# wkvong/multimodal-baby

Measured on AMD Instinct MI355X. Metric: image-text pairs/sec, CVCL ResNeXt+embed 224², bs256, 1/2/4/8 MI355X, higher is better.
Workload: dtype bf16; 1 GPU; C2 = BASELINE configs[1]: CVCL saycam_contrastive, frozen random-init ResNeXt-50 32x4d (BN train mode) + embedding mean-pool text encoder, E=512, L2-normalised, fixed tau 0.07, 224x224 frames + 3-word utterances; full step = fwd + InfoNCE + bwd(fc, embedding) + AdamW; per_gpu_batch=256, global_batch=256, negatives=local (single GPU), parallelism=dp1, trunk_streams=2

## Files before the change

include/cvcl_hip.h:

```cpp
#ifndef CVCL_HIP_H
#define CVCL_HIP_H

#include <stddef.h>
#include <stdint.h>

#ifdef __cplusplus
extern "C" {
#endif

#define CVCL_ABI_VERSION 7

enum { CVCL_OK = 0, CVCL_EINVAL = -1, CVCL_ELAUNCH = -2, CVCL_EWORKSPACE = -3, CVCL_EUNSUPPORTED = -4 };
enum { CVCL_F32 = 0, CVCL_BF16 = 1, CVCL_F32X3 = 2 };
enum { CVCL_ACT_NONE = 0, CVCL_ACT_RELU = 1, CVCL_ACT_GELU = 2, CVCL_ACT_QUICK_GELU = 3 };
#define CVCL_STATS_ACCUMULATE (-1)

int cvcl_abi_version(void);
const char* cvcl_last_error(void);

enum { CVCL_K_GEMM = 0, CVCL_K_GCONV = 1, CVCL_K_STEM = 2, CVCL_K_BN_FINALIZE = 3, CVCL_K_BN_ADD_RELU = 4,
       CVCL_K_MAXPOOL = 5, CVCL_K_AVGPOOL = 6, CVCL_K_HEAD = 7, CVCL_K_OTHER = 8, CVCL_K_ATTENTION = 9,
       CVCL_K_LAYERNORM = 10, CVCL_K_LSTM = 11, CVCL_K_GEMM_F32 = 12, CVCL_K_BN_APPLY = 13, CVCL_K_BN_BWD = 14,
       CVCL_K_WGRAD = 15, CVCL_K_GEMM8W = 16, CVCL_K_GEMM_PRO = 17, CVCL_K_NCLASSES = 18 };
int cvcl_prof_enable(int on);
// ... 21 lines not shown
                             void* stream);

size_t cvcl_infonce_workspace_bytes(int N);
int cvcl_infonce_fwd(const float* logits, int N, float* scalars5, float* row_lse, float* col_lse,
                     void* workspace, size_t workspace_bytes, void* stream);
int cvcl_infonce_bwd(const float* logits, const float* row_lse, const float* col_lse, const float* d_loss,
                     float* d_logits, int N, void* stream);

int cvcl_row_entropy(const float* x, float* out, int R, int N, void* stream);

typedef struct {
    const void* A; const void* W; void* C;
    int M, N, K, lda, ldw, ldc;
    const float* a_scale; const float* a_shift; int a_relu;
    int gather_ho, gather_wo, gather_hi, gather_wi, gather_stride;
    const float* exp_scale; const float* bias; int act;
    const void* R; int ldr;
    float* stats; int stats_rows;
    const float* c_scale; const float* c_shift; const float* r_scale; const float* r_shift;
    void* C_pre; const void* G; int ldg;
    const float* centre;
    const void* A2; const void* W2; int K2, lda2, ldw2; const float* centre2;
    const float* ln_stats; const float* ln_colsum; float* row_part;
    int a_trans, w_trans; float* a_rowsum;
    int f32_split;
} cvcl_gemm_args;
int cvcl_gemm_grid_m(int dtype, int M, int N, int has_prologue);
int cvcl_gemm(int dtype, const cvcl_gemm_args* args, void* stream);
int cvcl_gemm_stats_rows(int dtype, const cvcl_gemm_args* args);
int cvcl_gemm8w(int epi, const cvcl_gemm_args* args, void* stream);
int cvcl_gemm_pro(const cvcl_gemm_args* args, void* stream);
int cvcl_gemm_pro_supported(const cvcl_gemm_args* args);
int cvcl_gemm_pro_stats_rows(int M, int N);
int cvcl_gemm8w_supported(int M, int N, int K, int lda, int ldw, int ldc);
int cvcl_set_gemm_cu_share(int cus);
int cvcl_gemm_ln_supported(const cvcl_gemm_args* args);
int cvcl_row_stats(int dtype, const void* x, long x_row_stride, float* out, long rows, int D, float eps, void* stream);
int cvcl_row_stats_finalize(const float* row_part, int strips, float* out, long rows, int D, float eps, void* stream);
int cvcl_gemm8w_tile_rows(int M, int N);
int cvcl_gemm8w_stats_rows(int M, int N);

size_t cvcl_conv1x1_gram_workspace_bytes(int K);
int cvcl_conv1x1_gram(const void* A, int lda, long M, int K, const float* a_scale, const float* a_shift, int a_relu, void* workspace,
                      size_t workspace_bytes, const double** gram_out, void* stream);
int cvcl_bn_from_gram(const double* gram, int K, long count, const void* W, int ldw, int N, const float* gamma, const float* beta,
                      float* running_mean, float* running_var, int64_t* num_batches_tracked, float momentum, float eps,
                      float* scale, float* shift, float* moments, int moments_ld, const float* centre, void* stream);

int cvcl_transpose_f32(const float* in, float* out, int rows, int cols, void* stream);
int cvcl_colsum_f32(const float* dY, float* d_bias, int M, int N, void* stream);

enum { CVCL_PACK_DENSE = 0, CVCL_PACK_STEM7 = 1, CVCL_PACK_GCONV3 = 2 };

typedef struct {
    const void* w;
    const float* gamma; const float* beta;
    float* running_mean; float* running_var; int64_t* num_batches_tracked;
} cvcl_convbn_params;

int cvcl_bn_finalize(const float* stats, int rows, long count, const float* gamma, const float* beta,
                     float* running_mean, float* running_var, int64_t* num_batches_tracked, float momentum,
                     float eps, float* scale, float* shift, const float* centre, int C, void* stream);
int cvcl_bn_eval_affine(const float* gamma, const float* beta, const float* running_mean, const float* running_var,
                        float eps, float* scale, float* shift, const float* centre, int C, void* stream);
int cvcl_col_stats_rows(long rows);
int cvcl_col_stats(int dtype, const void* x, long rows, int C, float* stats, int stats_rows, void* stream);

size_t cvcl_packed_weight_bytes(int dtype, int kind, int cout, int cin_per_group, int k);
int cvcl_pack_conv_weight(int dtype, int kind, const float* w_oihw, void* out, int cout, int cin_per_group, int k,
                          void* stream);

int cvcl_stem_conv_stats_rows(int dtype, int B, int H, int W);
int cvcl_stem_conv7x7(int dtype, const float* x_nchw, const void* w_packed, void* y_nhwc, float* stats, int stats_rows,
                      const float* centre , int B, int H, int W, void* stream);
int cvcl_stem_pool_supported(int dtype, int H, int W);
int cvcl_stem_pool(int dtype, const float* x_nchw, const void* w_packed, const float* scale, const float* shift,
                   const float* centre , void* y_nhwc, int B, int H, int W, void* stream);
int cvcl_bn_relu_maxpool(int dtype, const void* x, const float* scale, const float* shift, void* y, int B, int H, int W,
                         int C, void* stream);
int cvcl_gconv3x3_stats_rows(int dtype, int B, int H, int W, int C, int stride);
int cvcl_gconv3x3(int dtype, const void* x, const float* a_scale, const float* a_shift, const void* w_packed, void* y,
                  float* stats, int stats_rows, const float* centre , int B, int H, int W, int C, int groups,
                  int stride, void* stream);
int cvcl_bn_add_relu(int dtype, const void* raw, const float* scale, const float* shift, const void* idn,
                     const float* idn_scale, const float* idn_shift, void* out, long rows, int C, void* stream);
int cvcl_bn_relu_apply(int dtype, const void* x, const float* scale, const float* shift, void* y, long rows, int C,
                       void* stream);
int cvcl_avgpool(int dtype, const void* x, float* out, int B, int HW, int C, void* stream);

size_t cvcl_resnext50_workspace_bytes(int dtype, int B, int H, int W);
size_t cvcl_resnext50_centres_floats(void);
int cvcl_resnext50_fwd(int dtype, int B, int H, int W, int training, const float* x_nchw,
                       const cvcl_convbn_params* layers, int n_layers, void* workspace, size_t workspace_bytes,
                       void* layer4_out_nhwc, float* pooled, float momentum, float eps, const float* centres, void* stream);
size_t cvcl_resnext50_block_workspace_bytes(int dtype, int B, int h, int w, int stage);
int cvcl_resnext50_block_fwd(int dtype, int B, int h, int w, int stage, int first, int training, const void* x_nhwc,
                             const cvcl_convbn_params* layers, int n_layers, void* workspace, size_t workspace_bytes,
                             void* out_nhwc, float momentum, float eps, const float* centres ,
                             void* stream);
size_t cvcl_resnext50_moments_floats(void);
int cvcl_resnext50_fwd_deferred_stats(int dtype, int B, int H, int W, const float* x_nchw,
                                      const cvcl_convbn_params* layers, int n_layers, void* workspace, size_t workspace_bytes,
                                      void* layer4_out_nhwc, float* pooled, float eps, float* moments, const float* centres,
                                      void* stream);
int cvcl_resnext50_apply_moments(const cvcl_convbn_params* layers, int n_layers, const float* moments, float momentum,
                                 void* stream);
size_t cvcl_resnext50_fwd_grouped_workspace_bytes(int dtype, int B, int H, int W, int group);
int cvcl_resnext50_fwd_grouped(int dtype, int B, int H, int W, int group, const float* x_nchw,
                               const cvcl_convbn_params* layers, int n_layers, void* workspace, size_t workspace_bytes,
                               void* layer4_out_nhwc, float* pooled, float eps, void* stream);

int cvcl_im2col_patches(int dtype, const float* x_nchw, void* cols, int B, int H, int W, int patch, int Kpad,
                        void* stream);
int cvcl_vit_assemble_tokens(int dtype, const void* tok, const float* cls, const float* pos, void* h, int B, int T,
                             int D, void* stream);
int cvcl_layernorm(int dtype, const void* x, long x_row_stride, const float* gamma, const float* beta, float eps,
                   void* y, int y_is_f32, long rows, int D, void* stream);
int cvcl_attention(int dtype, const void* qkv, const int64_t* key_tok, void* out, int B, int T, int heads, int head_dim,
                   float scale, void* stream);
int cvcl_attention_causal(int dtype, const void* qkv, void* out, int B, int T, int heads, int head_dim, float scale, void* stream);
int cvcl_clip_text_pool(const float* x, const int64_t* tok, const float* gamma, const float* beta, float eps, float* out, int B, int L,
                        int W, void* stream);
int cvcl_attention_mx(const void* qkv, void* out8, void* out_block_scales, int B, int T, int heads, int head_dim, float scale,
                      void* stream);
int cvcl_attention_train(const void* qkv, void* out, float* lse, int B, int T, int heads, int head_dim, float scale, void* stream);
int cvcl_attention_bwd(const void* qkv, const void* o, const void* d_o, const float* lse, void* d_qkv, int B, int T, int heads,
                       int head_dim, float scale, void* stream);
int cvcl_layernorm_bwd_rows_partials(long rows);
int cvcl_layernorm_bwd_rows(const void* x, long x_row_stride, const float* gamma, const void* dy, int dy_is_f32, long dy_row_stride,
                            float eps, const void* add, void* dx, long dx_row_stride, float* partial, long rows, int D, void* stream);
int cvcl_gelu_bf16(const void* u, const void* d_y, void* y, long n, void* stream);
int cvcl_vit_tokens_bwd(const void* dh, void* d_tok, float* d_pos, int B, int T, int D, void* stream);
int cvcl_attention_train_f32(const float* qkv, float* out, float* lse, int B, int T, int heads, int head_dim, float scale, void* stream);
int cvcl_attention_bwd_f32(const float* qkv, const float* o, const float* d_o, const float* lse, float* d_qkv, int B, int T, int heads,
                           int head_dim, float scale, void* stream);
int cvcl_layernorm_bwd_rows_f32(const float* x, long x_row_stride, const float* gamma, const float* dy, long dy_row_stride, float eps,
                                const float* add, float* dx, long dx_row_stride, float* partial, long rows, int D, void* stream);
int cvcl_gelu_f32(const float* u, const float* d_y, float* y, long n, void* stream);
int cvcl_vit_tokens_bwd_f32(const float* dh, float* d_tok, float* d_pos, int B, int T, int D, void* stream);
int cvcl_embed_gather_pos(const float* table, const int64_t* tok, const float* pos, float* x, int B, int L, int E, int V,
                          void* stream);
int cvcl_seq_sum_div(const float* x, const int64_t* len, float* ret, int B, int L, int E, void* stream);
int cvcl_lstm_cell(const float* gates, const int64_t* len, int t, float* h, float* c, float* out, int B, int L, int Hd,
                   void* stream);

int cvcl_dropout(const float* x, const float* residual, float* y, long n, float p, unsigned long long seed,
                 long shared_period, long inner, void* stream);
int cvcl_layernorm_bwd(const float* x, const float* gamma, const float* dy, float eps, float* dx, float* dy_xhat, long rows,
                       int D, void* stream);
int cvcl_relu_bwd(const float* y, const float* dy, float* dx, long n, void* stream);
int cvcl_embed_rows_bwd(const float* dx, const int64_t* tok, float* d_table, int n_pos, int E, int V, void* stream);
int cvcl_seq_sum_div_bwd(const float* d_ret, const int64_t* len, float* dx, int B, int L, int E, void* stream);
int cvcl_attention_small(const float* qkv, const int64_t* key_tok, const float* d_out, float* out, float* d_qkv, int B,
                         int T, int heads, int head_dim, float scale, float dropout_p, unsigned long long seed,
                         void* stream);
int cvcl_lstm_cell_train(const float* gates, const int64_t* len, int t, float* h, float* c, float* out ,
                         float* gates_act, float* c_save, float* h_prev_save, int B, int L, int Hd, void* stream);
int cvcl_lstm_cell_bwd(const float* gates_act, const float* c_save, const int64_t* len, int t, const float* dh, float* dc,
                       float* d_gates, float* dh_carry, int B, int L, int Hd, void* stream);

int cvcl_bn_apply(int dtype, const void* x, const float* scale, const float* shift, void* y, long rows, int C, int relu,
                  void* stream);
int cvcl_bn_bwd_partial_rows(int dtype, long rows, int C);
int cvcl_bn_bwd(int dtype, int mode, const void* x, const void* out, const void* dy, const float* scale, const float* shift,
                const float* mean, const float* rstd, const float* gamma, float* dgamma, float* dbeta, void* dx, void* g_out,
                long rows, int C, float* partial, int partial_rows, float* coef, void* stream);
// ... 138 lines not shown
```

multimodal-baby_amd/csrc/resnext.hip:

```cpp
#include <algorithm>
#include <array>
#include <cstdlib>
#include <type_traits>

#include "cvcl_common.h"

namespace {

constexpr int kMaxStatsRows = 1024;
constexpr size_t kTrunkAccLayer = (size_t)kBnAccRows * 2 * 2048;


__global__ __launch_bounds__(1024) void bn_finalize_kernel(const float* __restrict__ stats, int rows, double count,
                                                           const float* __restrict__ gamma, const float* __restrict__ beta,
                                                           float* __restrict__ running_mean, float* __restrict__ running_var,
                                                           int64_t* __restrict__ nbt, float momentum, float eps,
                                                           float* __restrict__ scale, float* __restrict__ shift, int C,
                                                           float* __restrict__ moments, int moments_ld,
                                                           const float* __restrict__ centre) {
    constexpr int NS = 64, NC = 16;
    __shared__ double ps[NS][NC], pq[NS][NC];
    const int c = threadIdx.x & (NC - 1), sl = threadIdx.x / NC, ch = blockIdx.x * NC + c;
    double s = 0.0, q = 0.0;
    if (ch < C) {
// ... 663 lines not shown
    f32x4 acc_init = {0.f, 0.f, 0.f, 0.f};
    if (p.centre) {
        const f32x4 cv = *reinterpret_cast<const f32x4*>(p.centre + c0 + wave * 16 + kb * 4);
        acc_init = f32x4{-cv[0], -cv[1], -cv[2], -cv[3]};
    }
    const int n_items = p.B * p.bands;
    const int st_off = (tid >> 3) * p.C + (tid & 7) * 8;
    __builtin_amdgcn_s_waitcnt(0x0F70);
    const int bx = (gridDim.x & 7) == 0 ? (int)((blockIdx.x & 7) * (gridDim.x >> 3) + (blockIdx.x >> 3)) : (int)blockIdx.x;
    if (bx < n_items) prefetch(bx);
    for (int item = bx; item < n_items; item += gridDim.x) {
        const int b = item / p.bands, band = item - b * p.bands;
        const int oy0 = band * p.TH;
        __syncthreads();
        auto stage = [&](auto RELU) __attribute__((always_inline)) {
#pragma unroll
            for (int i = 0; i < NPF; ++i) {
                const int pi = s_pix0 + 32 * i;
                const unsigned keep = pf_in[i] ? 0xffffffffu : 0u;
                u32x4 v;
#pragma unroll
                for (int e = 0; e < 4; ++e) {
                    unsigned y = round2(__builtin_elementwise_fma(widen2(pf[i][e]), sc[e], sh[e]));
                    if constexpr (decltype(RELU)::value) y = relu2(y);
                    v[e] = y & keep;
                }
                if (pi < npix_in) *reinterpret_cast<u32x4*>(smem + pi * GC_PIXB + s_chunk * 16) = v;
            }
        };
        if (relu_in) stage(std::true_type{});
        else stage(std::false_type{});
        __syncthreads();
        if (item + (int)gridDim.x < n_items) prefetch(item + gridDim.x);
        const int rows_left = p.Ho - oy0;
#pragma unroll
        for (int mt = 0; mt < NMT; mt += 2) {
            if (mt >= n_mt) break;
            const int e0 = mtab[mt], e1 = mtab[mt + 1];
            const int base0 = e0 & 0xffff, base1 = e1 & 0xffff;
            const int q0 = pix + 16 * mt, q1 = q0 + 16;
            const bool wr0 = (e0 >> 24) && ((e0 >> 16) & 0xff) < rows_left, wr1 = (e1 >> 24) && ((e1 >> 16) & 0xff) < rows_left;
            f32x4 acc0 = acc_init, acc1 = acc_init;
#pragma unroll
            for (int ks = 0; ks < KS; ++ks) {
                const bf16x8 a0 = *reinterpret_cast<const bf16x8*>(smem + base0 + tap_off[ks]);
                const bf16x8 a1 = *reinterpret_cast<const bf16x8*>(smem + base1 + tap_off[ks]);
                acc0 = __builtin_amdgcn_mfma_f32_16x16x32_bf16(wf[ks], a0, acc0, 0, 0, 0);
                acc1 = __builtin_amdgcn_mfma_f32_16x16x32_bf16(wf[ks], a1, acc1, 0, 0, 0);
            }
            if (wr0) {
                const u32x2 o = {round2(f32x2{acc0[0], acc0[1]}), round2(f32x2{acc0[2], acc0[3]})};
                *reinterpret_cast<u32x2*>(s_out + q0 * GC_PIXB + wave * 32 + kb * 8) = o;
#pragma unroll
                for (int e = 0; e < 2; ++e) { const f32x2 sv = widen2(o[e]); ssum[e] += sv; ssq[e] = __builtin_elementwise_fma(sv, sv, ssq[e]); }
            }
            if (wr1) {
                const u32x2 o = {round2(f32x2{acc1[0], acc1[1]}), round2(f32x2{acc1[2], acc1[3]})};
                *reinterpret_cast<u32x2*>(s_out + q1 * GC_PIXB + wave * 32 + kb * 8) = o;
#pragma unroll
                for (int e = 0; e < 2; ++e) { const f32x2 sv = widen2(o[e]); ssum[e] += sv; ssq[e] = __builtin_elementwise_fma(sv, sv, ssq[e]); }
            }
        }
        __syncthreads();
        const int valid_rows = min(p.TH, p.Ho - oy0);
        const int n_chunks = valid_rows * p.Wo * 8;
        bf16_t* yb = y + ((long)b * p.Ho + oy0) * p.Wo * p.C + c0 + st_off;
        const char* so = s_out + (tid >> 3) * GC_PIXB + (tid & 7) * 16;
#pragma unroll
        for (int k = 0; k < NMT / 2; ++k) {
            if (tid + 256 * k < n_chunks)
                *reinterpret_cast<bf16x8*>(yb + (long)k * 32 * p.C) = *reinterpret_cast<const bf16x8*>(so + k * 32 * GC_PIXB);
        }
    }
#pragma unroll
    for (int e = 0; e < 4; ++e) {
        float s = ssum[e >> 1][e & 1], q = ssq[e >> 1][e & 1];
#pragma unroll
        for (int o = 1; o < 16; o <<= 1) { s += __shfl_xor(s, o, 64); q += __shfl_xor(q, o, 64); }
        if (pix == 0 && p.stats) {
            const int ch = c0 + wave * 16 + kb * 4 + e;
            cvcl_bn_stats_out(p.stats, p.stats_acc, blockIdx.x, p.C, ch, s, q);
        }
    }
}

__global__ __launch_bounds__(256) void gconv_direct_f32_kernel(const float* __restrict__ x, const float* __restrict__ a_scale,
                                                               const float* __restrict__ a_shift, const float* __restrict__ w,
                                                               float* __restrict__ y, const float* __restrict__ centre,
                                                               int B, int H, int W, int C, int cg,
                                                               int stride, int Ho, int Wo, float act_floor) {
    const long total = (long)B * Ho * Wo * C;
    for (long i = (long)blockIdx.x * blockDim.x + threadIdx.x; i < total; i += (long)gridDim.x * blockDim.x) {
        const int co = (int)(i % C);
        const long pp = i / C;
        const int ox = (int)(pp % Wo), oy = (int)((pp / Wo) % Ho), b = (int)(pp / ((long)Wo * Ho));
        const int g0 = (co / cg) * cg;
        float acc = centre ? -centre[co] : 0.f;
        for (int ci = 0; ci < cg; ++ci) {
            const float sc = a_scale ? a_scale[g0 + ci] : 1.f, sh = a_scale ? a_shift[g0 + ci] : 0.f;
            for (int ky = 0; ky < 3; ++ky) {
                const int yin = oy * stride - 1 + ky;
                if (yin < 0 || yin >= H) continue;
                for (int kx = 0; kx < 3; ++kx) {
                    const int xin = ox * stride - 1 + kx;
                    if (xin < 0 || xin >= W) continue;
                    const float v = fmaxf(fmaf(x[(((long)b * H + yin) * W + xin) * C + g0 + ci], sc, sh), act_floor);
                    acc = fmaf(v, w[((long)co * cg + ci) * 9 + ky * 3 + kx], acc);
                }
            }
        }
        y[i] = acc;
    }
}

template <int CG>
__global__ __launch_bounds__(256) void gconv_tiled_f32_kernel(const float* __restrict__ x, const float* __restrict__ a_scale,
                                                              const float* __restrict__ a_shift, const float* __restrict__ w,
                                                              float* __restrict__ y, const float* __restrict__ centre,
                                                              int B, int H, int W, int C, int stride, int Ho, int Wo, int TH,
                                                              int bands, int plane_p, float act_floor) {
    extern __shared__ __attribute__((aligned(16))) float smf[];
    constexpr int NG = 64 / CG;
    const int Wp = W + 2, rows_in = (TH - 1) * stride + 3, plane = rows_in * Wp;
    float* ws = smf;
    float* cs = ws + 64 * 9 * CG;
    float* xs = cs + 64;
    const int c0 = blockIdx.y * 64;
    const int tid = threadIdx.x, lane = tid & 63;
    const int wave = __builtin_amdgcn_readfirstlane(tid >> 6);
    for (int e = tid; e < 64 * CG * 9; e += 256) {
        const int co = e / (CG * 9), r = e - co * (CG * 9), ci = r / 9, tap = r - ci * 9;
        const int g = co / CG, o = co - g * CG;
        ws[((g * 9 + tap) * CG + ci) * CG + o] = w[(long)c0 * CG * 9 + e];
    }
    if (tid < 64) cs[tid] = centre ? -centre[c0 + tid] : 0.f;
    const int ch4 = tid & 15;
    f32x4 sc4 = {1.f, 1.f, 1.f, 1.f}, sh4 = {0.f, 0.f, 0.f, 0.f};
    if (a_scale) {
        sc4 = *reinterpret_cast<const f32x4*>(a_scale + c0 + ch4 * 4);
        sh4 = *reinterpret_cast<const f32x4*>(a_shift + c0 + ch4 * 4);
    }
    for (int item = blockIdx.x; item < B * bands; item += gridDim.x) {
        const int b = item / bands, band = item - b * bands;
        const int oy0 = band * TH, iy0 = oy0 * stride - 1;
        __syncthreads();
        for (int pix = tid >> 4; pix < plane; pix += 16) {
            const int ry = pix / Wp, rx = pix - ry * Wp;
            const int yin = iy0 + ry, xin = rx - 1;
            f32x4 v = {0.f, 0.f, 0.f, 0.f};
            if ((unsigned)yin < (unsigned)H && (unsigned)xin < (unsigned)W) {
                v = *reinterpret_cast<const f32x4*>(x + (((long)b * H + yin) * W + xin) * C + c0 + ch4 * 4);
                if (a_scale) {
#pragma unroll
                    for (int k = 0; k < 4; ++k) v[k] = fmaxf(fmaf(v[k], sc4[k], sh4[k]), act_floor);
                }
            }
#pragma unroll
            for (int k = 0; k < 4; ++k) xs[(ch4 * 4 + k) * plane_p + pix] = v[k];
        }
        __syncthreads();
        const int n_out = min(TH, Ho - oy0) * Wo, nblk = (n_out + 63) / 64;
        for (int u = wave; u < NG * nblk; u += 4) {
            const int g = u / nblk, blk = u - g * nblk;
            const int q = blk * 64 + lane;
            const bool ok = q < n_out;
            const int qq = ok ? q : 0, ty = qq / Wo, ox = qq - ty * Wo;
// ... 388 lines not shown
                       "cvcl_stem_conv7x7: width %d not supported by the staged patch", W);
        const int g = stem_grid(B, H);
        CVCL_CHECK_ARG(!stats || stats_rows >= g, "cvcl_stem_conv7x7: stats_rows %d < %d", stats_rows, g);
        const size_t lds = (size_t)3 * STEM_ROWS * STEM_PITCH * 4 + 4 * 16 * STEM_OPITCH + 64 * 4;
        float* st = stats;
        CVCL_CHECK_ARG(st, "cvcl_stem_conv7x7: the bf16 kernel always emits statistics; pass a buffer");
        CvclProfScope prof(stream, CVCL_K_STEM);
        hipLaunchKernelGGL(stem_mfma_kernel, dim3(g), dim3(256), lds, s, x_nchw, (const bf16_t*)w_packed, (bf16_t*)y_nhwc,
                           st, centre, B, H, W);
        CVCL_LAUNCH_CHECK();
        return CVCL_OK;
    }
    const long total = (long)B * (H / 2) * (W / 2) * 64;
    {
        CvclProfScope prof(stream, CVCL_K_STEM);
        const int Ho = H / 2;
        auto lds_of = [&](int th) { return (size_t)(147 * 64 + 64 + 3 * (2 * th + 5) * (W + 6)) * 4; };
        int TH = Ho < 8 ? Ho : 8;
        while (TH > 1 && lds_of(TH) > 150 * 1024) --TH;
        if (lds_of(TH) <= 150 * 1024) {
            static CvclLdsAttr attr;
            if (const int rc = cvcl_raise_lds_limit(attr, (const void*)stem_tiled_f32_kernel, 160 * 1024, "cvcl_stem_conv7x7")) return rc;
            attr.mark();
            const int bands = cvcl_div_up(Ho, TH);
            const long items = (long)B * bands;
            hipLaunchKernelGGL(stem_tiled_f32_kernel, dim3((unsigned)(items < 1024 ? items : 1024)), dim3(256), lds_of(TH), s, x_nchw,
                               (const float*)w_packed, (float*)y_nhwc, centre, B, H, W, TH, bands);
        } else {
            hipLaunchKernelGGL(stem_direct_f32_kernel, dim3(cvcl_grid(total, 256, 8192)), dim3(256), 0, s, x_nchw,
                               (const float*)w_packed, (float*)y_nhwc, centre, B, H, W);
        }
    }
    CVCL_LAUNCH_CHECK();
    if (stats) return cvcl_col_stats(CVCL_F32, y_nhwc, (long)B * (H / 2) * (W / 2), 64, stats, stats_rows, stream);
    return CVCL_OK;
}

extern "C" int cvcl_stem_pool_supported(int dtype, int H, int W) {
    return dtype == CVCL_BF16 && H % 2 == 0 && W % 4 == 0 && W / 4 <= 64 && W + 6 + 8 <= 2 * STEM_PITCH && W / 2 + 2 <= STEMP_BW;
}

extern "C" int cvcl_stem_pool(int dtype, const float* x_nchw, const void* w_packed, const float* scale, const float* shift,
                              const float* centre, void* y_nhwc, int B, int H, int W, void* stream) {
    CVCL_CHECK_DTYPE(dtype, "cvcl_stem_pool");
    CVCL_CHECK_ARG(x_nchw && w_packed && scale && shift && y_nhwc && B > 0, "cvcl_stem_pool: bad args");
    CVCL_CHECK_ARG(cvcl_stem_pool_supported(dtype, H, W), "cvcl_stem_pool: bf16 and a width <= %d only (got dtype %d, %d x %d)",
                   2 * (STEMP_BW - 2), dtype, H, W);
    const size_t lds = (size_t)3 * STEMP_ROWS * STEM_PITCH * 4 + (size_t)STEMP_CR * STEMP_BW * 128 + 3 * 64 * 4;
    static CvclLdsAttr attr;
    if (const int rc = cvcl_raise_lds_limit(attr, (const void*)stem_pool_mfma_kernel, (int)lds, "cvcl_stem_pool")) return rc;
    attr.mark();
    const int Hp = (H / 2 - 1) / 2 + 1;
    const int items = B * cvcl_div_up(Hp, STEMP_TP);
    int dev = 0, cus = 256;
    if (hipGetDevice(&dev) != hipSuccess || hipDeviceGetAttribute(&cus, hipDeviceAttributeMultiprocessorCount, dev) != hipSuccess || cus <= 0) cus = 256;
    const int grid = items < cus ? items : cus;
    CvclProfScope prof(stream, CVCL_K_STEM);
    hipLaunchKernelGGL(stem_pool_mfma_kernel, dim3(grid), dim3(512), lds, (hipStream_t)stream, x_nchw, (const bf16_t*)w_packed,
                       (bf16_t*)y_nhwc, scale, shift, centre, B, H, W);
    CVCL_LAUNCH_CHECK();
    return CVCL_OK;
}

extern "C" int cvcl_bn_relu_maxpool(int dtype, const void* x, const float* scale, const float* shift, void* y, int B,
                                    int H, int W, int C, void* stream) {
    CVCL_CHECK_DTYPE_TRUNK(dtype, "cvcl_bn_relu_maxpool");
    dtype = cvcl_storage_dtype(dtype);
    CVCL_CHECK_ARG(x && scale && shift && y && C % 8 == 0, "cvcl_bn_relu_maxpool: bad args");
    CvclProfScope prof(stream, CVCL_K_MAXPOOL);
    const int Ho = (H - 1) / 2 + 1, Wo = (W - 1) / 2 + 1;
    const long total = (long)B * ((Ho + POOL_ROWS - 1) / POOL_ROWS) * Wo * (C / 8);
    const int grid = cvcl_grid(total, 256, 8192);
    if (dtype == CVCL_F32)
        hipLaunchKernelGGL(bn_relu_maxpool_kernel<float>, dim3(grid), dim3(256), 0, (hipStream_t)stream,
                           (const float*)x, scale, shift, (float*)y, B, H, W, C);
    else
        hipLaunchKernelGGL(bn_relu_maxpool_kernel<bf16_t>, dim3(grid), dim3(256), 0, (hipStream_t)stream,
                           (const bf16_t*)x, scale, shift, (bf16_t*)y, B, H, W, C);
    CVCL_LAUNCH_CHECK();
    return CVCL_OK;
}

namespace {
struct GconvPlan { int TH, bands, rows_in, grid_x; size_t lds; };
GconvPlan gconv_plan(int B, int H, int W, int C, int stride) {
    GconvPlan g;
    const int Ho = (H - 1) / stride + 1, Wo = (W - 1) / stride + 1, Wp = W + 2;
    auto bytes = [&](int th) { return (size_t)(((th - 1) * stride + 3) * Wp + th * Wo) * GC_PIXB; };
    int TH = Ho;
    while (TH > 1 && (bytes(TH) > (size_t)52 * 1024 || ((TH - 1) * stride + 3) * Wp > 10 * 32 || TH * Wo > 128)) TH = (TH + 1) / 2;
    g.TH = TH;
    g.bands = cvcl_div_up(Ho, TH);
    g.rows_in = (TH - 1) * stride + 3;
    g.lds = bytes(TH);
    int per_cu = (int)((160 * 1024) / g.lds);
    const int reg_limit = (C / 32 == 32) ? 2 : 3;
    if (per_cu > reg_limit) per_cu = reg_limit;
    if (per_cu < 1) per_cu = 1;
    const int slabs = C / GC_CS;
    int gx = per_cu * 256 / slabs;
    if (gx < 1) gx = 1;
    const int items = B * g.bands;
    g.grid_x = items < gx ? items : gx;
    return g;
}
}

extern "C" int cvcl_gconv3x3_stats_rows(int dtype, int B, int H, int W, int C, int stride) {
    if (!cvcl_dtype_trunk(dtype)) return 0;
    if (dtype == CVCL_F32X3) return C % 32 == 0 ? cvcl_gconv_split_stats_rows(B, H, W, C, stride) : 0;
    if (dtype == CVCL_BF16) return gconv_plan(B, H, W, C, stride).grid_x;
    const int Ho = (H - 1) / stride + 1, Wo = (W - 1) / stride + 1;
    return cvcl_col_stats_rows((long)B * Ho * Wo);
}

static int gconv3x3_impl(int dtype, const void* x, const float* a_scale, const float* a_shift, const BnSrc* src, const void* w_packed,
                         void* y, float* stats, int stats_rows, const float* centre, int B, int H, int W, int C, int groups,
                         int stride, void* stream) {
    CVCL_CHECK_DTYPE_TRUNK(dtype, "cvcl_gconv3x3");
    CVCL_CHECK_ARG(x && w_packed && y && (!a_scale == !a_shift), "cvcl_gconv3x3: null pointer");
    CVCL_CHECK_ARG(!src || (dtype == CVCL_BF16 && src->acc && src->gamma && src->beta && src->C == C && src->count > 0 &&
                            (const void*)src->acc != (const void*)stats),
                   "cvcl_gconv3x3: finalize-on-load source");
    CVCL_CHECK_ARG(stats_rows != CVCL_STATS_ACCUMULATE || dtype == CVCL_BF16, "cvcl_gconv3x3: accumulators exist for bf16 only");
    const float act_floor = (a_scale || src) ? 0.f : -INFINITY;
    CVCL_CHECK_ARG(B > 0 && (stride == 1 || stride == 2) && groups > 0 && C % groups == 0, "cvcl_gconv3x3: bad shape");
    const int cg = C / groups;
    const int Ho = (H - 1) / stride + 1, Wo = (W - 1) / stride + 1;
    hipStream_t s = (hipStream_t)stream;
    if (dtype == CVCL_F32X3)
        return cvcl_gconv_split((const float*)x, a_scale, a_shift, act_floor, w_packed, (float*)y, stats, stats_rows, centre, B, H, W, C,
                                cg, stride, stream);
    if (dtype == CVCL_BF16) {
        CVCL_CHECK_ARG((cg == 4 || cg == 8 || cg == 16 || cg == 32) && C % GC_CS == 0,
                       "cvcl_gconv3x3: unsupported channels-per-group %d (C=%d)", cg, C);
        const GconvPlan g = gconv_plan(B, H, W, C, stride);
        CVCL_CHECK_ARG(g.lds <= 160 * 1024 && g.rows_in * (W + 2) <= 10 * 32 && g.TH * ((W - 1) / stride + 1) <= 128,
                       "cvcl_gconv3x3: feature map too wide for one staged band (%zu B, %d pixels)", g.lds, g.rows_in * (W + 2));
        CVCL_CHECK_ARG(!stats || stats_rows == CVCL_STATS_ACCUMULATE || stats_rows >= g.grid_x, "cvcl_gconv3x3: stats_rows %d < %d", stats_rows, g.grid_x);
        GconvDev d;
        d.x = x; d.a_scale = a_scale; d.a_shift = a_shift; d.w = w_packed; d.y = y; d.stats = stats; d.centre = centre;
        d.B = B; d.H = H; d.W = W; d.C = C; d.cg = cg; d.stride = stride; d.Ho = Ho; d.Wo = Wo;
        d.TH = g.TH; d.bands = g.bands; d.rows_in = g.rows_in;
        d.act_floor = act_floor;
        d.src = BnSrc{};
        d.stats_acc = stats && stats_rows == CVCL_STATS_ACCUMULATE;
        if (src) {
            CVCL_CHECK_ARG(g.lds >= 2048, "cvcl_gconv3x3: band buffers smaller than the finalize-on-load scratch");
            d.src = *src;
        }
        CvclProfScope prof(stream, CVCL_K_GCONV);
        int rc;
        const int slots = cvcl_div_up(g.rows_in * (W + 2), 32);
        static CvclLdsAttr attr_set[2][2][11];
        auto launch = [&](auto kern) -> int {
            CvclLdsAttr& done = attr_set[cg == 32][g.TH * Wo <= 64][slots <= 4 ? 4 : slots <= 6 ? 6 : slots <= 8 ? 8 : 10];
            if (const int rc = cvcl_raise_lds_limit(done, (const void*)kern, 160 * 1024, "cvcl_gconv3x3")) return rc;
            done.mark();
            hipLaunchKernelGGL(kern, dim3(g.grid_x, C / GC_CS), dim3(256), g.lds, s, d);
            return CVCL_OK;
        };
        const bool few = g.TH * Wo <= 64;
#define CVCL_GCONV_PICK(W_) \
        (slots <= 4 ? (few ? launch(gconv_mfma_kernel<W_, 4, 4>) : launch(gconv_mfma_kernel<W_, 4, 8>)) \
         : slots <= 6 ? (few ? launch(gconv_mfma_kernel<W_, 6, 4>) : launch(gconv_mfma_kernel<W_, 6, 8>)) \
         : slots <= 8 ? (few ? launch(gconv_mfma_kernel<W_, 8, 4>) : launch(gconv_mfma_kernel<W_, 8, 8>)) \
                      : (few ? launch(gconv_mfma_kernel<W_, 10, 4>) : launch(gconv_mfma_kernel<W_, 10, 8>)))
        rc = cg == 32 ? CVCL_GCONV_PICK(true) : CVCL_GCONV_PICK(false);
#undef CVCL_GCONV_PICK
        if (rc) return rc;
        CVCL_LAUNCH_CHECK();
        return CVCL_OK;
    }
    const long total = (long)B * Ho * Wo * C;
    {
        CvclProfScope prof(stream, CVCL_K_GCONV);
        auto plane_p_of = [&](int th) { const int pl = ((th - 1) * stride + 3) * (W + 2); return pl + ((9 - (pl & 7)) & 7); };
        auto lds_of = [&](int th) { return (size_t)(64 * 9 * cg + 64 + 64 * plane_p_of(th)) * 4; };
        int TH = Ho;
        while (TH > 1 && lds_of(TH) > 150 * 1024) --TH;
        const bool tiled = C % 64 == 0 && (cg == 4 || cg == 8 || cg == 16 || cg == 32) && lds_of(TH) <= 150 * 1024 &&
                           ((uintptr_t)x & 15) == 0 && ((uintptr_t)y & 15) == 0 && ((uintptr_t)a_scale & 15) == 0 && ((uintptr_t)a_shift & 15) == 0;
        if (tiled) {
            const int bands = cvcl_div_up(Ho, TH);
            const long items = (long)B * bands;
            const int slabs = C / 64;
            long gx = 1024 / slabs;
            if (gx < 1) gx = 1;
            if (gx > items) gx = items;
            static CvclLdsAttr attr[4];
            auto launch = [&](auto kern, int slot) -> int {
                if (const int rc = cvcl_raise_lds_limit(attr[slot], (const void*)kern, 160 * 1024, "cvcl_gconv3x3")) return rc;
                attr[slot].mark();
                hipLaunchKernelGGL(kern, dim3((unsigned)gx, slabs), dim3(256), lds_of(TH), s, (const float*)x, a_scale, a_shift,
                                   (const float*)w_packed, (float*)y, centre, B, H, W, C, stride, Ho, Wo, TH, bands, plane_p_of(TH), act_floor);
                return CVCL_OK;
            };
            const int rc = cg == 4 ? launch(gconv_tiled_f32_kernel<4>, 0) : cg == 8 ? launch(gconv_tiled_f32_kernel<8>, 1)
                         : cg == 16 ? launch(gconv_tiled_f32_kernel<16>, 2) : launch(gconv_tiled_f32_kernel<32>, 3);
            if (rc) return rc;
        } else {
            hipLaunchKernelGGL(gconv_direct_f32_kernel, dim3(cvcl_grid(total, 256, 8192)), dim3(256), 0, s, (const float*)x, a_scale,
                               a_shift, (const float*)w_packed, (float*)y, centre, B, H, W, C, cg, stride, Ho, Wo, act_floor);
        }
    }
    CVCL_LAUNCH_CHECK();
    if (stats) return cvcl_col_stats(CVCL_F32, y, (long)B * Ho * Wo, C, stats, stats_rows, stream);
    return CVCL_OK;
}

extern "C" int cvcl_gconv3x3(int dtype, const void* x, const float* a_scale, const float* a_shift, const void* w_packed,
                             void* y, float* stats, int stats_rows, const float* centre, int B, int H, int W, int C, int groups,
                             int stride, void* stream) {
    return gconv3x3_impl(dtype, x, a_scale, a_shift, nullptr, w_packed, y, stats, stats_rows, centre, B, H, W, C, groups, stride, stream);
}

extern "C" int cvcl_bn_add_relu(int dtype, const void* raw, const float* scale, const float* shift, const void* idn,
                                const float* idn_scale, const float* idn_shift, void* out, long rows, int C, void* stream) {
    CVCL_CHECK_DTYPE_TRUNK(dtype, "cvcl_bn_add_relu");
    dtype = cvcl_storage_dtype(dtype);
    CVCL_CHECK_ARG(raw && scale && shift && idn && out && rows > 0 && C % 8 == 0, "cvcl_bn_add_relu: bad args");
    CvclProfScope prof(stream, CVCL_K_BN_ADD_RELU);
    CVCL_CHECK_ARG((idn_scale == nullptr) == (idn_shift == nullptr), "cvcl_bn_add_relu: idn_scale/idn_shift pair");
    const int epc = dtype == CVCL_F32 ? 4 : 8;
    CVCL_CHECK_ARG(C % epc == 0, "cvcl_bn_add_relu: C must be a multiple of %d", epc);
    hipStream_t s = (hipStream_t)stream;
    const int cc = C / epc;
    int g256 = cc, t256 = 256;
    while (t256) { const int r = g256 % t256; g256 = t256; t256 = r; }
    const int mult = cc / g256;
    int grid = cvcl_grid(rows * (long)cc, 256 * 4, 16384);
    grid = (grid + mult - 1) / mult * mult;
    if (dtype == CVCL_F32)
        hipLaunchKernelGGL(bn_add_relu_kernel<float>, dim3(grid), dim3(256), 0, s, (const float*)raw,
                           scale, shift, (const float*)idn, idn_scale, idn_shift, (float*)out, rows, C);
    else
        hipLaunchKernelGGL(bn_add_relu_kernel<bf16_t>, dim3(grid), dim3(256), 0, s, (const bf16_t*)raw,
                           scale, shift, (const bf16_t*)idn, idn_scale, idn_shift, (bf16_t*)out, rows, C);
    CVCL_LAUNCH_CHECK();
    return CVCL_OK;
}

extern "C" int cvcl_bn_relu_apply(int dtype, const void* x, const float* scale, const float* shift, void* y, long rows,
                                  int C, void* stream) {
    CVCL_CHECK_DTYPE_TRUNK(dtype, "cvcl_bn_relu_apply");
    dtype = cvcl_storage_dtype(dtype);
    CVCL_CHECK_ARG(x && scale && shift && y && rows > 0, "cvcl_bn_relu_apply: bad args");
    CvclProfScope prof(stream, CVCL_K_BN_APPLY);
    const int epc = dtype == CVCL_F32 ? 4 : 8;
    CVCL_CHECK_ARG(C % epc == 0, "cvcl_bn_relu_apply: C must be a multiple of %d", epc);
    const int cc = C / epc;
    int g256 = cc, t256 = 256;
    while (t256) { const int r = g256 % t256; g256 = t256; t256 = r; }
    const int mult = cc / g256;
    int grid = cvcl_grid(rows * (long)cc, 256 * 4, 16384);
    grid = (grid + mult - 1) / mult * mult;
    if (dtype == CVCL_F32)
        hipLaunchKernelGGL(bn_relu_apply_kernel<float>, dim3(grid), dim3(256), 0, (hipStream_t)stream, (const float*)x, scale,
                           shift, (float*)y, rows, C);
    else
        hipLaunchKernelGGL(bn_relu_apply_kernel<bf16_t>, dim3(grid), dim3(256), 0, (hipStream_t)stream, (const bf16_t*)x,
                           scale, shift, (bf16_t*)y, rows, C);
    CVCL_LAUNCH_CHECK();
    return CVCL_OK;
}

extern "C" int cvcl_avgpool(int dtype, const void* x, float* out, int B, int HW, int C, void* stream) {
    CVCL_CHECK_DTYPE_TRUNK(dtype, "cvcl_avgpool");
    dtype = cvcl_storage_dtype(dtype);
    CVCL_CHECK_ARG(x && out && B > 0 && HW > 0 && C > 0, "cvcl_avgpool: bad args");
    CvclProfScope prof(stream, CVCL_K_AVGPOOL);
    if (dtype == CVCL_F32)
        hipLaunchKernelGGL(avgpool_kernel<float>, dim3(cvcl_grid((long)B * C, 256, 4096)), dim3(256), 0, (hipStream_t)stream, (const float*)x, out, B, HW, C);
    else
        hipLaunchKernelGGL(avgpool_kernel<bf16_t>, dim3(cvcl_grid((long)B * C, 256, 4096)), dim3(256), 0, (hipStream_t)stream, (const bf16_t*)x, out, B, HW, C);
    CVCL_LAUNCH_CHECK();
    return CVCL_OK;
}

namespace {
constexpr int kLayers[4] = {3, 4, 6, 3};
constexpr int kTrunkLayers = 53;
constexpr int kMaxC = 2048;
constexpr int kAffStride = 2 * kMaxC;
enum { kConv1, kConv2, kConv3, kDownsample };
static_assert(sizeof(EvalAffineAll::C) == sizeof(int) * kTrunkLayers && sizeof(ApplyMomentsAll::C) == sizeof(int) * kTrunkLayers,
              "the one-launch layer tables hold the whole trunk");

constexpr int block_layer_c(int stage, int j) { return (64 << stage) * (j < kConv3 ? 2 : 4); }

constexpr std::array<int, kTrunkLayers> kTrunkC = [] {
    std::array<int, kTrunkLayers> c = {64};
    int l = 1;
    for (int st = 0; st < 4; ++st)
        for (int b = 0; b < kLayers[st]; ++b)
            for (int j = 0; j < (b == 0 ? 4 : 3); ++j) c[l++] = block_layer_c(st, j);
    return c;
}();

// ... 454 lines not shown
```

Measured before the change: 51110 pairs/s.

## Add warp-specialized producer/consumer pipelined grouped 3x3 conv kernel

Adds a 512-thread grouped-conv kernel in which 256 threads load, apply the input BN affine, and stage the next band into double-buffered LDS, while the other 256 threads run MFMA on the current band and write outputs to a separate buffer that the producers store. It is chosen by default for stride-1 shapes 28/256, 14/512 and 7/1024. The intent is to overlap global loads and stores with MFMA compute and hide memory latency. In exchange the kernel needs more LDS per block, uses smaller bands, and allows fewer resident blocks per CU.

```diff
diff --git a/include/cvcl_hip.h b/include/cvcl_hip.h
--- a/include/cvcl_hip.h
+++ b/include/cvcl_hip.h
@@ -127,6 +127,12 @@
 int cvcl_gconv3x3(int dtype, const void* x, const float* a_scale, const float* a_shift, const void* w_packed, void* y,
                   float* stats, int stats_rows, const float* centre , int B, int H, int W, int C, int groups,
                   int stride, void* stream);
+int cvcl_gconv3x3_planned_form(int H, int W, int C, int stride);
+int cvcl_gconv3x3_form_stats_rows(int form, int B, int H, int W, int C, int stride);
+int cvcl_gconv3x3_form(int form, const void* x, const float* a_scale, const float* a_shift, const int64_t* src_acc,
+                       const float* src_gamma, const float* src_beta, double src_count, float src_eps, const void* w_packed, void* y,
+                       float* stats, int stats_rows, const float* centre , int B, int H, int W, int C, int groups,
+                       int stride, void* stream);
 int cvcl_bn_add_relu(int dtype, const void* raw, const float* scale, const float* shift, const void* idn,
                      const float* idn_scale, const float* idn_shift, void* out, long rows, int C, void* stream);
 int cvcl_bn_relu_apply(int dtype, const void* x, const float* scale, const float* shift, void* y, long rows, int C,
diff --git a/multimodal-baby_amd/csrc/resnext.hip b/multimodal-baby_amd/csrc/resnext.hip
--- a/multimodal-baby_amd/csrc/resnext.hip
+++ b/multimodal-baby_amd/csrc/resnext.hip
@@ -769,6 +769,210 @@
             cvcl_bn_stats_out(p.stats, p.stats_acc, blockIdx.x, p.C, ch, s, q);
         }
     }
+}
+
+__host__ __device__ constexpr int gcp_barriers(int n_items_of_workgroup) { return n_items_of_workgroup + 1; }
+constexpr int GCP_OUTB = 128;
+
+template <bool WIDE, int NMT>
+__device__ __forceinline__ void gcp_consumer(const GconvDev& p, char* smem, int tid, int bx, int n_local, int in_bytes, int out_bytes) {
+    const int lane = tid & 63, wave = tid >> 6;
+    const int pix = lane & 15, kb = lane >> 4;
+    const int c0 = blockIdx.y * GC_CS;
+    const int Wp = p.W + 2;
+    constexpr bool wide = WIDE;
+    constexpr int KS = WIDE ? 9 : 5;
+    const int unit = c0 / 16 + wave;
+    const bf16_t* wu = (const bf16_t*)p.w + (long)unit * KS * 512;
+    bf16x8 wf[KS];
+#pragma unroll
+    for (int ks = 0; ks < KS; ++ks) wf[ks] = *reinterpret_cast<const bf16x8*>(wu + (ks * 16 + pix) * 32 + kb * 8);
+    const int in_ch_off = wide ? ((wave >> 1) * 32 + kb * 8) : (wave * 16 + (kb & 1) * 8);
+    f32x2 ssum[2] = {f32x2{0.f, 0.f}, f32x2{0.f, 0.f}}, ssq[2] = {f32x2{0.f, 0.f}, f32x2{0.f, 0.f}};
+    const int n_out = p.TH * p.Wo, n_mt = cvcl_div_up(n_out, 16);
+    int tap_off[KS];
+#pragma unroll
+    for (int ks = 0; ks < KS; ++ks) {
+        int tap = wide ? ks : 2 * ks + (kb >> 1);
+        if (tap > 8) tap = 8;
+        const int ky = tap / 3, kx = tap - ky * 3;
+        tap_off[ks] = (ky * Wp + kx) * GC_PIXB + in_ch_off * 2;
+    }
+    int mtab[NMT];
+#pragma unroll
+    for (int mt = 0; mt < NMT; ++mt) {
+        const int q = pix + 16 * mt;
+        const bool ok = mt < n_mt && q < n_out;
+        const int ty = q / p.Wo, ox = q - ty * p.Wo;
+        mtab[mt] = ok ? ((((ty * p.stride) * Wp + ox * p.stride) * GC_PIXB) | (ty << 16) | (1 << 24)) : 0;
+    }
+    f32x4 acc_init = {0.f, 0.f, 0.f, 0.f};
+    if (p.centre) {
+        const f32x4 cv = *reinterpret_cast<const f32x4*>(p.centre + c0 + wave * 16 + kb * 4);
+        acc_init = f32x4{-cv[0], -cv[1], -cv[2], -cv[3]};
+    }
+    const int out_off = pix * GCP_OUTB + (((wave * 2 + (kb >> 1)) ^ ((pix >> 1) & 7)) << 4) + (kb & 1) * 8;
+    const int nb = gcp_barriers(n_local);
+    for (int j = 0; j < nb; ++j) {
+        if (j >= 1) {
+            const int k = j - 1, item = bx + k * (int)gridDim.x;
+            const int band = item % p.bands, oy0 = band * p.TH;
+            const char* s_in = smem + (k & 1) * in_bytes;
+            char* s_out = smem + 2 * in_bytes + (k & 1) * out_bytes + out_off;
+            const int rows_left = p.Ho - oy0;
+#pragma unroll
+            for (int mt = 0; mt < NMT; mt += 2) {
+                if (mt >= n_mt) break;
+                const int e0 = mtab[mt], e1 = mtab[mt + 1];
+                const int base0 = e0 & 0xffff, base1 = e1 & 0xffff;
+                const bool wr0 = (e0 >> 24) && ((e0 >> 16) & 0xff) < rows_left, wr1 = (e1 >> 24) && ((e1 >> 16) & 0xff) < rows_left;
+                f32x4 acc0 = acc_init, acc1 = acc_init;
+#pragma unroll
+                for (int ks = 0; ks < KS; ++ks) {
+                    const bf16x8 a0 = *reinterpret_cast<const bf16x8*>(s_in + base0 + tap_off[ks]);
+                    const bf16x8 a1 = *reinterpret_cast<const bf16x8*>(s_in + base1 + tap_off[ks]);
+                    acc0 = __builtin_amdgcn_mfma_f32_16x16x32_bf16(wf[ks], a0, acc0, 0, 0, 0);
+                    acc1 = __builtin_amdgcn_mfma_f32_16x16x32_bf16(wf[ks], a1, acc1, 0, 0, 0);
+                }
+                if (wr0) {
+                    const u32x2 o = {round2(f32x2{acc0[0], acc0[1]}), round2(f32x2{acc0[2], acc0[3]})};
+                    *reinterpret_cast<u32x2*>(s_out + 16 * mt * GCP_OUTB) = o;
+#pragma unroll
+                    for (int e = 0; e < 2; ++e) { const f32x2 sv = widen2(o[e]); ssum[e] += sv; ssq[e] = __builtin_elementwise_fma(sv, sv, ssq[e]); }
+                }
+                if (wr1) {
+                    const u32x2 o = {round2(f32x2{acc1[0], acc1[1]}), round2(f32x2{acc1[2], acc1[3]})};
+                    *reinterpret_cast<u32x2*>(s_out + 16 * (mt + 1) * GCP_OUTB) = o;
+#pragma unroll
+                    for (int e = 0; e < 2; ++e) { const f32x2 sv = widen2(o[e]); ssum[e] += sv; ssq[e] = __builtin_elementwise_fma(sv, sv, ssq[e]); }
+                }
+            }
+        }
+        __syncthreads();
+    }
+#pragma unroll
+    for (int e = 0; e < 4; ++e) {
+        float s = ssum[e >> 1][e & 1], q = ssq[e >> 1][e & 1];
+#pragma unroll
+        for (int o = 1; o < 16; o <<= 1) { s += __shfl_xor(s, o, 64); q += __shfl_xor(q, o, 64); }
+        if (pix == 0 && p.stats) {
+            const int ch = c0 + wave * 16 + kb * 4 + e;
+            cvcl_bn_stats_out(p.stats, p.stats_acc, blockIdx.x, p.C, ch, s, q);
+        }
+    }
+}
+
+template <int NPF, int NMT>
+__device__ __forceinline__ void gcp_producer(const GconvDev& p, char* smem, int tid, int bx, int n_local, int in_bytes, int out_bytes,
+                                             const float* aff) {
+    const bf16_t* __restrict__ x = (const bf16_t*)p.x;
+    bf16_t* __restrict__ y = (bf16_t*)p.y;
+    const int c0 = blockIdx.y * GC_CS;
+    const int Wp = p.W + 2;
+    const int s_chunk = tid & 7, s_pix0 = tid >> 3;
+    f32x2 sc[4], sh[4];
+#pragma unroll
+    for (int e = 0; e < 4; ++e) {
+        const int cl = s_chunk * 8 + 2 * e, ch = c0 + cl;
+        if (aff) {
+            sc[e] = f32x2{aff[cl], aff[cl + 1]};
+            sh[e] = f32x2{aff[64 + cl], aff[64 + cl + 1]};
+        } else {
+            sc[e] = p.a_scale ? f32x2{p.a_scale[ch], p.a_scale[ch + 1]} : f32x2{1.f, 1.f};
+            sh[e] = p.a_scale ? f32x2{p.a_shift[ch], p.a_shift[ch + 1]} : f32x2{0.f, 0.f};
+        }
+    }
+    const bool relu_in = p.act_floor == 0.f;
+    const int npix_in = p.rows_in * Wp;
+    u32x4 pf[NPF];
+    bool pf_in[NPF];
+    int slot_y[NPF], slot_xoff[NPF];
+    bool slot_ok[NPF];
+#pragma unroll
+    for (int i = 0; i < NPF; ++i) {
+        const int pi = s_pix0 + 32 * i;
+        const int pc = min(pi, npix_in - 1);
+        const int ry = pc / Wp, xin = pc - ry * Wp - 1;
+        slot_y[i] = ry;
+        slot_ok[i] = pi < npix_in && xin >= 0 && xin < p.W;
+        slot_xoff[i] = min(max(xin, 0), p.W - 1) * p.C;
+    }
+    const int row_elems = p.W * p.C;
+    auto prefetch = [&](int item) {
+        const int b = item / p.bands, band = item - b * p.bands;
+        const int iy0 = band * p.TH * p.stride - 1;
+        const bf16_t* xb = x + (long)b * p.H * p.W * p.C + c0 + s_chunk * 8;
+#pragma unroll
+        for (int i = 0; i < NPF; ++i) {
+            const int yin = iy0 + slot_y[i];
+            pf_in[i] = slot_ok[i] && (unsigned)yin < (unsigned)p.H;
+            const int yc = min(max(yin, 0), p.H - 1);
+            pf[i] = *reinterpret_cast<const u32x4*>(xb + (yc * row_elems + slot_xoff[i]));
+        }
+    };
+    auto stage = [&](char* s_in, auto RELU) __attribute__((always_inline)) {
+#pragma unroll
+        for (int i = 0; i < NPF; ++i) {
+            const int pi = s_pix0 + 32 * i;
+            const unsigned keep = pf_in[i] ? 0xffffffffu : 0u;
+            u32x4 v;
+#pragma unroll
+            for (int e = 0; e < 4; ++e) {
+                unsigned y = round2(__builtin_elementwise_fma(widen2(pf[i][e]), sc[e], sh[e]));
+                if constexpr (decltype(RELU)::value) y = relu2(y);
+                v[e] = y & keep;
+            }
+            if (pi < npix_in) *reinterpret_cast<u32x4*>(s_in + pi * GC_PIXB + s_chunk * 16) = v;
+        }
+    };
+    const int st_off = (tid >> 3) * p.C + (tid & 7) * 8;
+    const int so_off = (tid >> 3) * GCP_OUTB + (((tid & 7) ^ ((tid >> 4) & 7)) << 4);
+    auto store = [&](int k) {
+        const int item = bx + k * (int)gridDim.x;
+        const int b = item / p.bands, band = item - b * p.bands;
+        const int oy0 = band * p.TH;
+        const int valid_rows = min(p.TH, p.Ho - oy0);
+        const int n_chunks = valid_rows * p.Wo * 8;
+        bf16_t* yb = y + ((long)b * p.Ho + oy0) * p.Wo * p.C + c0 + st_off;
+        const char* so = smem + 2 * in_bytes + (k & 1) * out_bytes + so_off;
+#pragma unroll
+        for (int kk = 0; kk < NMT / 2; ++kk) {
+            if (tid + 256 * kk < n_chunks)
+                *reinterpret_cast<bf16x8*>(yb + (long)kk * 32 * p.C) = *reinterpret_cast<const bf16x8*>(so + kk * 32 * GCP_OUTB);
+        }
+    };
+    if (n_local > 0) prefetch(bx);
+    const int nb = gcp_barriers(n_local);
+    for (int j = 0; j < nb; ++j) {
+        if (j < n_local) {
+            char* s_in = smem + (j & 1) * in_bytes;
+            if (relu_in) stage(s_in, std::true_type{});
+            else stage(s_in, std::false_type{});
+            if (j + 1 < n_local) prefetch(bx + (j + 1) * (int)gridDim.x);
+        }
+        if (j >= 2) store(j - 2);
+        __syncthreads();
+    }
+    if (nb >= 2) store(nb - 2);
+}
+
+template <bool WIDE, int NPF, int NMT>
+__global__ __launch_bounds__(512, NPF <= 6 ? 4 : 2) void gconv_mfma_pipe_kernel(GconvDev p) {
+    extern __shared__ __attribute__((aligned(16))) char smem[];
+    const int tid = threadIdx.x;
+    const int c0 = blockIdx.y * GC_CS;
+    const float* aff = nullptr;
+    if (p.src.acc) {
+        float* a = reinterpret_cast<float*>(smem + 2 * p.rows_in * (p.W + 2) * GC_PIXB);
+        bn_slice_affine<GC_CS>(p.src, c0, blockIdx.x == 0, a, a + 64);
+        aff = a;
+    }
+    const int bx = (gridDim.x & 7) == 0 ? (int)((blockIdx.x & 7) * (gridDim.x >> 3) + (blockIdx.x >> 3)) : (int)blockIdx.x;
+    const int n_items = p.B * p.bands;
+    const int n_local = bx < n_items ? (n_items - bx + (int)gridDim.x - 1) / (int)gridDim.x : 0;
+    const int in_bytes = p.rows_in * (p.W + 2) * GC_PIXB, out_bytes = p.TH * p.Wo * GCP_OUTB;
+    if (tid < 256) gcp_consumer<WIDE, NMT>(p, smem, tid, bx, n_local, in_bytes, out_bytes);
+    else gcp_producer<NPF, NMT>(p, smem, tid - 256, bx, n_local, in_bytes, out_bytes, aff);
 }
 
 __global__ __launch_bounds__(256) void gconv_direct_f32_kernel(const float* __restrict__ x, const float* __restrict__ a_scale,
@@ -1323,19 +1527,28 @@
 }
 
 namespace {
-struct GconvPlan { int TH, bands, rows_in, grid_x; size_t lds; };
-GconvPlan gconv_plan(int B, int H, int W, int C, int stride) {
+enum { GCONV_ONE_PHASE = 0, GCONV_PIPELINED = 1, GCONV_FORM_OF_PLAN = -1 };
+struct GconvPlan { int TH, bands, rows_in, grid_x, form; size_t lds; };
+bool gconv_pipelined_wins(int H, int W, int C, int stride) {
+    return stride == 1 && H == W && ((H == 28 && C == 256) || (H == 14 && C == 512) || (H == 7 && C == 1024));
+}
+GconvPlan gconv_plan(int B, int H, int W, int C, int stride, int form = GCONV_FORM_OF_PLAN) {
     GconvPlan g;
     const int Ho = (H - 1) / stride + 1, Wo = (W - 1) / stride + 1, Wp = W + 2;
     auto bytes = [&](int th) { return (size_t)(((th - 1) * stride + 3) * Wp + th * Wo) * GC_PIXB; };
     int TH = Ho;
     while (TH > 1 && (bytes(TH) > (size_t)52 * 1024 || ((TH - 1) * stride + 3) * Wp > 10 * 32 || TH * Wo > 128)) TH = (TH + 1) / 2;
+    g.form = form == GCONV_FORM_OF_PLAN ? (gconv_pipelined_wins(H, W, C, stride) ? GCONV_PIPELINED : GCONV_ONE_PHASE) : form;
+    auto bytes_pipe = [&](int th) { return 2 * ((size_t)((th - 1) * stride + 3) * Wp * GC_PIXB + (size_t)th * Wo * GCP_OUTB); };
+    if (g.form == GCONV_PIPELINED)
+        while (TH > 1 && (bytes_pipe(TH) > (size_t)80 * 1024 || ((TH - 1) * stride + 3) * Wp > 6 * 32)) TH = (TH + 1) / 2;
     g.TH = TH;
     g.bands = cvcl_div_up(Ho, TH);
     g.rows_in = (TH - 1) * stride + 3;
-    g.lds = bytes(TH);
+    g.lds = g.form == GCONV_PIPELINED ? bytes_pipe(TH) : bytes(TH);
     int per_cu = (int)((160 * 1024) / g.lds);
-    const int reg_limit = (C / 32 == 32) ? 2 : 3;
+    const int reg_limit = g.form == GCONV_PIPELINED ? (cvcl_div_up(g.rows_in * Wp, 32) <= 6 ? 2 : 1)
+                        : (C / 32 == 32) ? 2 : 3;
     if (per_cu > reg_limit) per_cu = reg_limit;
     if (per_cu < 1) per_cu = 1;
     const int slabs = C / GC_CS;
@@ -1357,7 +1570,7 @@
 
 static int gconv3x3_impl(int dtype, const void* x, const float* a_scale, const float* a_shift, const BnSrc* src, const void* w_packed,
                          void* y, float* stats, int stats_rows, const float* centre, int B, int H, int W, int C, int groups,
-                         int stride, void* stream) {
+                         int stride, void* stream, int form = GCONV_FORM_OF_PLAN) {
     CVCL_CHECK_DTYPE_TRUNK(dtype, "cvcl_gconv3x3");
     CVCL_CHECK_ARG(x && w_packed && y && (!a_scale == !a_shift), "cvcl_gconv3x3: null pointer");
     CVCL_CHECK_ARG(!src || (dtype == CVCL_BF16 && src->acc && src->gamma && src->beta && src->C == C && src->count > 0 &&
@@ -1375,7 +1588,7 @@
     if (dtype == CVCL_BF16) {
         CVCL_CHECK_ARG((cg == 4 || cg == 8 || cg == 16 || cg == 32) && C % GC_CS == 0,
                        "cvcl_gconv3x3: unsupported channels-per-group %d (C=%d)", cg, C);
-        const GconvPlan g = gconv_plan(B, H, W, C, stride);
+        const GconvPlan g = gconv_plan(B, H, W, C, stride, form);
         CVCL_CHECK_ARG(g.lds <= 160 * 1024 && g.rows_in * (W + 2) <= 10 * 32 && g.TH * ((W - 1) / stride + 1) <= 128,
                        "cvcl_gconv3x3: feature map too wide for one staged band (%zu B, %d pixels)", g.lds, g.rows_in * (W + 2));
         CVCL_CHECK_ARG(!stats || stats_rows == CVCL_STATS_ACCUMULATE || stats_rows >= g.grid_x, "cvcl_gconv3x3: stats_rows %d < %d", stats_rows, g.grid_x);
@@ -1393,22 +1606,26 @@
         CvclProfScope prof(stream, CVCL_K_GCONV);
         int rc;
         const int slots = cvcl_div_up(g.rows_in * (W + 2), 32);
-        static CvclLdsAttr attr_set[2][2][11];
+        static CvclLdsAttr attr_set[2][2][2][11];
+        const bool pipelined = g.form == GCONV_PIPELINED;
+        CVCL_CHECK_ARG(!pipelined || !src || (size_t)g.TH * Wo * GCP_OUTB >= 512, "cvcl_gconv3x3: output band smaller than the finalize-on-load scratch");
         auto launch = [&](auto kern) -> int {
-            CvclLdsAttr& done = attr_set[cg == 32][g.TH * Wo <= 64][slots <= 4 ? 4 : slots <= 6 ? 6 : slots <= 8 ? 8 : 10];
+            CvclLdsAttr& done = attr_set[pipelined][cg == 32][g.TH * Wo <= 64][slots <= 4 ? 4 : slots <= 6 ? 6 : slots <= 8 ? 8 : 10];
             if (const int rc = cvcl_raise_lds_limit(done, (const void*)kern, 160 * 1024, "cvcl_gconv3x3")) return rc;
             done.mark();
-            hipLaunchKernelGGL(kern, dim3(g.grid_x, C / GC_CS), dim3(256), g.lds, s, d);
+            hipLaunchKernelGGL(kern, dim3(g.grid_x, C / GC_CS), dim3(pipelined ? 512 : 256), g.lds, s, d);
             return CVCL_OK;
         };
         const bool few = g.TH * Wo <= 64;
-#define CVCL_GCONV_PICK(W_) \
-        (slots <= 4 ? (few ? launch(gconv_mfma_kernel<W_, 4, 4>) : launch(gconv_mfma_kernel<W_, 4, 8>)) \
-         : slots <= 6 ? (few ? launch(gconv_mfma_kernel<W_, 6, 4>) : launch(gconv_mfma_kernel<W_, 6, 8>)) \
-         : slots <= 8 ? (few ? launch(gconv_mfma_kernel<W_, 8, 4>) : launch(gconv_mfma_kernel<W_, 8, 8>)) \
-                      : (few ? launch(gconv_mfma_kernel<W_, 10, 4>) : launch(gconv_mfma_kernel<W_, 10, 8>)))
+#define CVCL_GCONV_PICK_OF(K_, W_) \
+        (slots <= 4 ? (few ? launch(K_<W_, 4, 4>) : launch(K_<W_, 4, 8>)) \
+         : slots <= 6 ? (few ? launch(K_<W_, 6, 4>) : launch(K_<W_, 6, 8>)) \
+         : slots <= 8 ? (few ? launch(K_<W_, 8, 4>) : launch(K_<W_, 8, 8>)) \
+                      : (few ? launch(K_<W_, 10, 4>) : launch(K_<W_, 10, 8>)))
+#define CVCL_GCONV_PICK(W_) (pipelined ? CVCL_GCONV_PICK_OF(gconv_mfma_pipe_kernel, W_) : CVCL_GCONV_PICK_OF(gconv_mfma_kernel, W_))
         rc = cg == 32 ? CVCL_GCONV_PICK(true) : CVCL_GCONV_PICK(false);
 #undef CVCL_GCONV_PICK
+#undef CVCL_GCONV_PICK_OF
         if (rc) return rc;
         CVCL_LAUNCH_CHECK();
         return CVCL_OK;
@@ -1456,6 +1673,23 @@
     return gconv3x3_impl(dtype, x, a_scale, a_shift, nullptr, w_packed, y, stats, stats_rows, centre, B, H, W, C, groups, stride, stream);
 }
 
+extern "C" int cvcl_gconv3x3_form_stats_rows(int form, int B, int H, int W, int C, int stride) {
+    if (form != GCONV_ONE_PHASE && form != GCONV_PIPELINED) return 0;
+    return gconv_plan(B, H, W, C, stride, form).grid_x;
+}
+extern "C" int cvcl_gconv3x3_planned_form(int H, int W, int C, int stride) { return gconv_plan(1, H, W, C, stride).form; }
+extern "C" int cvcl_gconv3x3_form(int form, const void* x, const float* a_scale, const float* a_shift, const int64_t* src_acc,
+                                  const float* src_gamma, const float* src_beta, double src_count, float src_eps, const void* w_packed,
+                                  void* y, float* stats, int stats_rows, const float* centre, int B, int H, int W, int C, int groups,
+                                  int stride, void* stream) {
+    CVCL_CHECK_ARG(form == GCONV_ONE_PHASE || form == GCONV_PIPELINED, "cvcl_gconv3x3_form: form %d", form);
+    CVCL_CHECK_ARG(!src_acc || (!a_scale && !a_shift), "cvcl_gconv3x3_form: an affine and a finalize-on-load source");
+    BnSrc src{};
+    if (src_acc) { src.acc = reinterpret_cast<const long long*>(src_acc); src.gamma = src_gamma; src.beta = src_beta; src.count = src_count; src.eps = src_eps; src.C = C; }
+    return gconv3x3_impl(CVCL_BF16, x, a_scale, a_shift, src_acc ? &src : nullptr, w_packed, y, stats, stats_rows, centre, B, H, W, C,
+                         groups, stride, stream, form);
+}
+
 extern "C" int cvcl_bn_add_relu(int dtype, const void* raw, const float* scale, const float* shift, const void* idn,
                                 const float* idn_scale, const float* idn_shift, void* out, long rows, int C, void* stream) {
     CVCL_CHECK_DTYPE_TRUNK(dtype, "cvcl_bn_add_relu");
```

Result: no change. 51170 pairs/s, median of 3 (+0.1%).
